# LeadRDRK/ZPack

Measured on AMD Instinct MI355X. Metric: decompressed GiB/s over all entries; % HBM roofline, higher is better.
Workload: dtype u8; 1 GPU; c2_lz4_64k; entries_per_gpu=100000, entries_total=100000, archive_image_bytes_this_rank=3543588472, archive_image_bytes_all_ranks=3543588472, method=lz4, level=0, class_mix=70/20/5/5 text/records/random/runs, parallelism=one batch per rank, no data-path collective, rehearsal_one_card=False, frames_by=liblz4/libzstd of the image, reference writer call sequence

## Files before the change

zpack_amd/csrc/lz4_wave.h:

```cpp
#pragma once
#include "zpk_device.h"
#include "xxh3_device.h"
#include "seq_exec.h"

namespace zpk {

__device__ __noinline__ u32 window_word(const u8* a, const u8* lo, const u8* hi)
{
    if (a >= lo && a + 4 <= hi) return ld32(a);
    u32 v = 0;
    #pragma unroll
    for (int i = 0; i < 4; i++) if (a + i >= lo && a + i < hi) v |= (u32)ld8(a + i) << (8 * i);
    return v;
}

struct ByteWindow {
    u32 w;
    const u8* base;
    const u8* lo;
    const u8* hi;

    __device__ __forceinline__ void load(const u8* p, int lane)
    {
        base = (const u8*)((u64)p & ~(u64)3);
        w = window_word(base + 4 * lane, lo, hi);
    }
    __device__ __forceinline__ u32 byte(const u8* p, int lane)
    {
        u64 d = (u64)(p - base);
        if (d >= 256) { load(p, lane); d = (u64)(p - base); }
        u32 word = (u32)__builtin_amdgcn_readlane((int)w, (int)(d >> 2));
        return (word >> (8 * (d & 3))) & 0xFF;
    }
};

struct DecodeOut { int rc; u64 produced; };

struct Lz4Resume { u64 ip_off, op_off, frame_ip_off, frame_op_off; u32 in_blocks, nframes; };

#ifndef LZ4W_SEG
#define LZ4W_SEG 60u
#endif
static_assert(LZ4W_SEG <= 64u, "the visited-position mask of a segment is one 64-bit word");
#define LZ4W_CHUNK (64u * LZ4W_SEG)
#define LZ4W_SLACK 64u
#ifndef LZ4W_RUNIN
#define LZ4W_RUNIN LZ4W_SEG
#endif

#ifndef LZ4W_SPLIT_FIRST
#define LZ4W_SPLIT_FIRST 0
#endif
#ifndef LZ4W_NREC
#define LZ4W_NREC 576u
#endif
struct alignas(16) Lz4WaveShared {
    u8  stage[LZ4W_CHUNK + LZ4W_SLACK + 16];
    u16 rec[LZ4W_NREC];
};

struct Lz4Bytes {
    lds_cp8 S;
    const u8* g;
    u32 cbase, cend;
    __device__ __forceinline__ u32 at(u32 pos) const
    {
        if (pos < cend) return lds_ld8(S + (pos - cbase));
        return (u32)ld8(g + pos);
    }
    __device__ __forceinline__ u32 at16(u32 pos) const
    {
        if (pos + 1 < cend) return lds_ld16(S + (pos - cbase));
        return at(pos) | (at(pos + 1) << 8);
    }
};

struct Lz4Tok { u32 next, lit_pos, lit, ml, off, flags; };

__device__ __forceinline__ Lz4Tok lz4_token_at(const Lz4Bytes& B, u32 p, u32 C, bool want_offset)
{
    Lz4Tok t; t.flags = 0; t.ml = 0; t.off = 1;
    const u32 tok = B.at(p);
    u32 q = p + 1, lit = tok >> 4;
    if (lit == 15) {
        u32 b;
        do {
            if (q >= C) { t.flags = 1; t.next = C; t.lit = 0; t.lit_pos = q; return t; }
            b = B.at(q++); lit += b;
        } while (b == 255 && lit < 0x7F000000u);
        if (b == 255) { t.flags = 1; t.next = C; t.lit = 0; t.lit_pos = q; return t; }
    }
    t.lit_pos = q; t.lit = lit;
    if (lit > C - q) { t.flags = 1; t.next = C; return t; }
    q += lit;
    if (q == C) { t.flags = 2; t.next = C; return t; }
    if (C - q < 2) { t.flags = 5; t.next = C; return t; }
    if (want_offset) t.off = B.at16(q);
    q += 2;
    u32 ml = tok & 15;
    if (ml == 15) {
        u32 b;
        do {
            if (q >= C) { t.flags = 5; t.next = C; return t; }
            b = B.at(q++); ml += b;
        } while (b == 255 && ml < 0x7F000000u);
        if (b == 255) { t.flags = 5; t.next = C; return t; }
    }
    t.ml = ml + 4;
    t.next = q;
    return t;
}

struct Lz4Quick { u32 lit_pos, lit, ml, next, off, slow; };
__device__ __forceinline__ u32 lt31(u32 a, u32 b) { return (a - b) >> 31; }
__device__ __forceinline__ Lz4Quick lz4_quick(lds_cp8 S, u32 cbase, u32 p, u32 lim)
{
    const lds_cp8 at = S + (p - cbase);
    const u32 tok = lds_ld8(at), b1 = lds_ld8(at + 1);
    const u32 lit4 = tok >> 4, mlc = tok & 15;
    const u32 le = (lit4 + 1) >> 4, me = (mlc + 1) >> 4;
    const u32 lit = lit4 + (b1 & (0u - le));
    const u32 q = 1 + le + lit;
    const u32 b2 = lds_ld8(at + q + 2);
    Lz4Quick r;
    r.off = lds_ld16(at + q);
    r.lit_pos = p + 1 + le; r.lit = lit;
    r.ml = mlc + 4 + (b2 & (0u - me));
    r.next = p + q + 2 + me;
    r.slow = (le & ((b1 + 1) >> 8)) | (me & ((b2 + 1) >> 8)) | lt31(lim, p + q + 3);
    return r;
}

struct Lz4Walk { u32 exit, flags; u64 m; };
template <bool FIRST>
__device__ __forceinline__ Lz4Walk lz4_walk(const Lz4Bytes& B, bool on, u32 from, u32 seg_start, u32 seg_end, u32 C,
                                            const Lz4Walk& old, u32& entry_out, SeqStats& stt)
{
    (void)stt;
    const u32 lim = B.cend < C ? B.cend : C;
    const i32 seg_len = (i32)(seg_end - seg_start), lim_rel = (i32)(lim - seg_start);
    const lds_cp8 base = B.S + (seg_start - B.cbase);
    const bool start_in = on && (i32)(from - seg_start) < seg_len;
    i32 rp = start_in ? (i32)(from - seg_start) : seg_len;
    bool live = start_in, merged = false;
    u32 flags = 0, exit_far = from, far = on && !start_in ? 1u : 0u;
    u64 m = 0;
    for (;;) {
        live = live && rp < seg_len;
        const bool inseg = FIRST ? rp >= 0 : true;
        if (!FIRST) {
            const bool hit = live && ((u32)(old.m >> (rp & 63)) & 1u);
            merged = merged || hit;
            live = live && !hit;
        }
        if (__builtin_amdgcn_ballot_w64(live) == 0) break;
        SEQ_STAT(if (FIRST) stt.hops_first++; else stt.hops_fix++);
        m |= (u64)((live && inseg) ? 1u : 0u) << (rp & 63);
        const lds_cp8 at = base + rp;
        const u32 tok = lds_ld8(at), b1 = lds_ld8(at + 1);
        const u32 lit4 = tok >> 4, mlc = tok & 15;
        const bool l15 = lit4 == 15, m15 = mlc == 15;
        const u32 q = lit4 + 1 + (l15 ? b1 + 1 : 0u);
        const u32 b2 = lds_ld8(at + q + 2);
        const i32 n2 = rp + (i32)q + 2;
        i32 nx = n2 + (m15 ? 1 : 0);
        const bool slow = (l15 && b1 == 255) || (m15 && b2 == 255) || n2 >= lim_rel;
        if (live && slow) {
            SEQ_STAT(stt.slow_hops++);
            const Lz4Tok tt = lz4_token_at(B, seg_start + (u32)rp, C, false);
            nx = (i32)(tt.next - seg_start);
            if (tt.flags && !inseg) nx = 0;
            else if (tt.flags || nx >= seg_len) { flags |= tt.flags; far = 1; exit_far = tt.next; nx = seg_len; }
        }
        rp = live ? nx : rp;
    }
    Lz4Walk w; w.m = m; w.flags = flags; w.exit = far ? exit_far : seg_start + (u32)rp;
    if (merged) {
        const u64 tail = old.m & ~((1ull << (rp & 63)) - 1);
        w.m |= tail;
        w.flags |= old.flags;
        w.exit = old.exit;
    }
    if (!on) w = old;
    entry_out = !FIRST ? from : m ? seg_start + (u32)__ffsll((long long)m) - 1u : w.exit;
    return w;
}

struct Lz4NoEmit { __device__ __forceinline__ int operator()(const SeqBatch&, int, u32) const { return D_OK; } };

template <int COOP = 2, bool EMIT = false, class Emit = Lz4NoEmit>
__device__ inline int lz4_block_wave(Lz4WaveShared& sh, Watchdog& wd, SeqStats& stt, const u8* ip, u32 C, const u8* rd_hi,
                                     u8* dst_lo, u8*& op_io, u8* oend, int lane, Emit emit = Emit())
{
    u8* op = op_io;
    if (C == 0) return D_MALFORMED;
    u32 cpos = 0;
    bool finished = false;
    while (!finished) {
        if (wd.expired()) return D_MALFORMED;
        const u64 tp0 = SEQ_T(); (void)tp0;
        if (cpos >= C) return D_MALFORMED;
        const u32 nst = C - cpos < LZ4W_CHUNK + LZ4W_SLACK ? C - cpos : LZ4W_CHUNK + LZ4W_SLACK;
        const u32 tok_end = C - cpos < LZ4W_CHUNK ? C : cpos + LZ4W_CHUNK;
        wave_mem_fence();
        if (ip + cpos + ((nst + 15u) & ~15u) <= rd_hi) {
            const u8* const g = ip + cpos + 16u * (u32)lane;
            ZPK_LDS u8* const d0 = (ZPK_LDS u8*)sh.stage;
            #pragma unroll
            for (u32 i = 0; i < LZ4W_CHUNK + LZ4W_SLACK; i += WAVE * 16)
                if (i + 16u * (u32)lane < nst) __builtin_amdgcn_global_load_lds((const ZPK_GLOBAL u32*)(g + i), (ZPK_LDS u32*)(d0 + i), 16, 0, 0);
            asm volatile("s_waitcnt vmcnt(0)" ::: "memory");
        } else {
            for (u32 i = (u32)lane * 16; i < nst; i += WAVE * 16) {
                const u8* g = ip + cpos + i;
                if (i + 16 <= nst && g + 16 <= rd_hi) { u128 v = ld128(g); __builtin_memcpy(sh.stage + i, &v, 16); }
                else for (u32 k = i; k < nst && k < i + 16; k++) sh.stage[k] = ld8(ip + cpos + k);
            }
        }
        __builtin_amdgcn_fence(__ATOMIC_ACQ_REL, "workgroup");
        u64 ts = SEQ_T(); (void)ts; SEQ_STAT(stt.t_stage += ts - tp0; stt.chunks++);
        Lz4Bytes B; B.S = to_lds(sh.stage); B.g = ip; B.cbase = cpos; B.cend = cpos + nst;
        const u32 lim = B.cend < C ? B.cend : C;
        const u32 my_start = cpos + (u32)lane * LZ4W_SEG;
        const u32 my_end = my_start + LZ4W_SEG < tok_end ? my_start + LZ4W_SEG : tok_end;
        const bool active = my_start < tok_end;
        u32 my_entry = my_start;
        Lz4Walk w; w.exit = my_start; w.flags = 0; w.m = 0;
        w = lz4_walk<true>(B, active, lane == 0 ? my_start : (my_start - cpos > LZ4W_RUNIN ? my_start - LZ4W_RUNIN : cpos), my_start, my_end, C, w, my_entry, stt);
        SEQ_STAT({ u64 t2 = SEQ_T(); stt.t_walk1 += t2 - ts; ts = t2; });
        for (int iter = 0; iter < 66; iter++) {
            SEQ_STAT(stt.fix_iters++);
            u32 e = (u32)__shfl_up((int)w.exit, 1, 64);
            if (lane == 0) e = cpos;
            const bool changed = active && e != my_entry;
            if (__ballot(changed) == 0) break;
            u32 unused;
            w = lz4_walk<false>(B, changed, e, my_start, my_end, C, w, unused, stt);
            my_entry = changed ? e : my_entry;
        }
        SEQ_STAT({ u64 t2 = SEQ_T(); stt.t_fix += t2 - ts; ts = t2; });
        if (!active) { w.exit = (u32)__shfl((int)w.exit, 63, 64); }
        const u64 lastmask = __ballot(active);
        const int last_lane = 63 - __clzll((long long)lastmask);
        const u32 chain_exit = (u32)__builtin_amdgcn_readlane((int)w.exit, last_lane);
        const u32 fl = (u32)__ballot(active && (w.flags & 1)) != 0 || (__ballot(active && (w.flags & 1)) >> 32) != 0 ? 1u : 0u;
        if (__ballot(active && (w.flags & 2)) != 0) finished = true;
        const u32 my_nseq = active ? (u32)__popcll(w.m) : 0u;
        const u32 x = wave_scan_add(my_nseq);
        const u32 nseq = (u32)__builtin_amdgcn_readlane((int)x, 63);
        SEQ_STAT({ u64 t2 = SEQ_T(); stt.t_emit += t2 - ts; stt.t_parse += t2 - tp0; });
        ZPK_LDS u16* const rec = (ZPK_LDS u16*)sh.rec;
        for (u32 b0 = 0, bstep; b0 < nseq; b0 += bstep) {
            bstep = LZ4W_SPLIT_FIRST && b0 < WAVE ? WAVE / 2 : WAVE;
            const u32 bw = b0 % LZ4W_NREC;
            if (bw == 0) {
                wave_mem_fence();
                u64 m = w.m;
                u32 k = x - my_nseq;
                const u32 rel = my_start - cpos;
                while (m) {
                    const u32 b = (u32)__ffsll((long long)m) - 1u;
                    m &= m - 1;
                    if (k - b0 < LZ4W_NREC) rec[k - b0] = (u16)(rel + b);
                    k++;
                }
                if (active && x == nseq && nseq - b0 < LZ4W_NREC)
                    rec[nseq - b0] = (u16)(w.exit - cpos < LZ4W_CHUNK + LZ4W_SLACK ? w.exit - cpos : LZ4W_CHUNK + LZ4W_SLACK);
                wave_mem_fence();
            }
            const int cnt = (int)(nseq - b0 < bstep ? nseq - b0 : bstep);
            const u64 tq0 = SEQ_T(); (void)tq0;
            SeqBatch q; q.lit = ip; q.lit_lds = SEQ_NO_LDS; q.ll = 0; q.ml = 0; q.off = 1; q.bad = 0;
            u32 tok_pos = cpos;
            if (lane < cnt) {
                const u32 p = cpos + (u32)rec[bw + (u32)lane];
                tok_pos = p;
                const Lz4Quick t = lz4_quick(B.S, B.cbase, p, lim);
                if (!t.slow) {
                    q.lit = ip + t.lit_pos; q.ll = t.lit; q.ml = t.ml; q.off = t.off;
                } else {
                    const Lz4Tok tt = lz4_token_at(B, p, C, true);
                    q.lit = ip + tt.lit_pos; q.ll = tt.lit; q.ml = tt.ml; q.off = tt.off;
                    if (tt.flags & 1) q.bad = (tt.flags & 4) ? 2u : 1u;
                }
                if (q.ll > (1u << 23)) q.ll = 1u << 23;
                if (q.ml > (1u << 23)) q.ml = 1u << 23;
                const u32 lp = (u32)(q.lit - ip);
                if (q.ll <= SEQ_OWN_MAX && lp + q.ll <= B.cend) q.lit_lds = lp - B.cbase;
            }
            SEQ_STAT({ u64 t2 = SEQ_T(); stt.t_parse += t2 - tq0; stt.t_tok += t2 - tq0; });
            u32 dead = 0;
            if constexpr (!EMIT) {
                const u32 nx = bw + (u32)cnt;
                const u32 own = tok_pos - cpos;
#ifdef LZ4W_ROOM_OWN_TOKEN
                (void)nx; const u32 nxt = 0u;
#else
                const u32 nxt = (u32)rec[nx == LZ4W_NREC ? 0u : nx];
#endif
                dead = (u32)__builtin_amdgcn_readfirstlane((int)(nxt > own ? nxt : own));
            }
            int rc;
            if constexpr (EMIT) { (void)dead; rc = emit(q, cnt, (u32)(q.lit - ip)); }
            else rc = seq_exec_batch<true, COOP, SEQ_ASM_LONG_LIT != 0>(q, cnt, op, oend, dst_lo, -1, lane, stt, B.S, to_lds_rw(sh.stage), dead);
            if (rc != D_OK) { op_io = op; return rc; }
        }
        if (fl) return D_MALFORMED;
        if (!finished && chain_exit <= cpos) return D_MALFORMED;
        cpos = chain_exit;
    }
    if (cpos != C) return D_MALFORMED;
    op_io = op;
    return D_OK;
}

template <int COOP = 2>
__device__ inline DecodeOut lz4f_decode_wave(Lz4WaveShared& sh, Watchdog& wd, SeqStats& stt, const u8* src, u64 src_size, const u8* src_lo, const u8* src_hi,
                                             u8* dst, u64 dst_cap, int lane, Lz4Resume* rs = nullptr)
{
    DecodeOut r; r.rc = D_OK; r.produced = 0;
    const u8* ip = src;
    const u8* const iend = src + src_size;
    u8* op = dst;
    u8* const oend = dst + dst_cap;
    bool resume_in_blocks = false, first = true;
    if (rs && (rs->in_blocks || rs->nframes)) {
        ip = src + rs->frame_ip_off; op = dst + rs->frame_op_off;
        resume_in_blocks = rs->in_blocks != 0;
        first = rs->nframes == 0;
    }
    for (;; first = false) {
        if (wd.expired()) { r.rc = D_MALFORMED; return r; }
        if (!first && (ip == iend || op == oend)) break;
        if (rs) { rs->frame_ip_off = (u64)(ip - src); rs->frame_op_off = (u64)(op - dst); if (!resume_in_blocks) rs->in_blocks = 0; }
        if (iend - ip < 7) { r.rc = D_TRUNCATED; r.produced = (u64)(op - dst); return r; }
        const u32 magic = uld32(ip);
        if ((magic & 0xFFFFFFF0u) == 0x184D2A50u) {
            if (iend - ip < 8) { r.rc = D_TRUNCATED; r.produced = (u64)(op - dst); return r; }
            const u64 sz = uld32(ip + 4);
            if ((u64)(iend - ip) - 8 < sz) { r.rc = D_TRUNCATED; r.produced = (u64)(op - dst); return r; }
            ip += 8 + sz;
            if (rs) rs->nframes++;
            continue;
        }
        if (magic != 0x184D2204u) { r.rc = D_MALFORMED; return r; }
        const u32 flg = uld8(ip + 4), bd = uld8(ip + 5);
        const bool indep = (flg >> 5) & 1, bck = (flg >> 4) & 1, has_cs = (flg >> 3) & 1, cck = (flg >> 2) & 1, has_dict = flg & 1;
        if ((flg >> 6) != 1 || (flg & 2)) { r.rc = D_MALFORMED; return r; }
        const u32 hdr = 7 + (has_cs ? 8 : 0) + (has_dict ? 4 : 0);
        if ((u64)(iend - ip) < hdr) { r.rc = D_TRUNCATED; r.produced = (u64)(op - dst); return r; }
        if (bd & 0x8F) { r.rc = D_MALFORMED; return r; }
        const u32 bcode = (bd >> 4) & 7;
        if (bcode < 4) { r.rc = D_MALFORMED; return r; }
        const u64 bmax = (u64)1 << (8 + 2 * bcode);
        u64 content_size = 0;
        if (has_cs) content_size = uni64(ld64(ip + 6));
        {
            u32 h = 0;
            lane0_guard();
            if (lane == 0) h = (xxh32_serial(ip + 4, hdr - 5, 0) >> 8) & 0xFF;
            if (uni(h) != uld8(ip + hdr - 1)) { r.rc = D_MALFORMED; return r; }
        }
        ip += hdr;

        u8* const frame_out = op;
        if (resume_in_blocks) { ip = src + rs->ip_off; op = dst + rs->op_off; resume_in_blocks = false; }
        for (;;) {
            if (wd.expired()) { r.rc = D_MALFORMED; return r; }
            if (rs) { rs->in_blocks = 1; rs->ip_off = (u64)(ip - src); rs->op_off = (u64)(op - dst); }
            if (iend - ip < 4) { r.rc = D_TRUNCATED; r.produced = (u64)(op - dst); return r; }
            const u32 bh = uld32(ip);
            ip += 4;
            if (bh == 0) break;
            const bool raw = bh >> 31;
            const u64 bsz = bh & 0x7FFFFFFFu;
            if (bsz > bmax) { r.rc = D_MALFORMED; return r; }
            if ((u64)(iend - ip) < bsz + (bck ? 4u : 0u)) {
                if (raw && !rs) {
                    u64 n = (u64)(iend - ip); if (n > bsz) n = bsz;
                    bool full = n > (u64)(oend - op);
                    if (full) n = (u64)(oend - op);
                    for (u64 i = (u64)lane * 16; i < n; i += WAVE * 16) gcopy_upto16(op + i, ip + i, (u32)(n - i < 16 ? n - i : 16));
                    op += n;
                    if (full) { r.rc = D_DST_FULL; r.produced = (u64)(op - dst); return r; }
                }
                r.rc = D_TRUNCATED; r.produced = (u64)(op - dst); return r;
            }
            if (bck) {
                u32 h = 0;
                lane0_guard();
                if (lane == 0) h = xxh32_serial(ip, bsz, 0);
                if (uni(h) != uld32(ip + bsz)) { r.rc = D_MALFORMED; return r; }
            }
            if (raw) {
                u64 n = bsz;
                bool full = n > (u64)(oend - op);
                if (full) n = (u64)(oend - op);
                for (u64 i = (u64)lane * 16; i < n; i += WAVE * 16) gcopy_upto16(op + i, ip + i, (u32)(n - i < 16 ? n - i : 16));
                op += n;
                if (full) { r.rc = D_DST_FULL; r.produced = (u64)(op - dst); return r; }
            } else {
                u8* hist_lo = indep ? op : frame_out;
                if ((u64)(op - hist_lo) > 65536) hist_lo = op - 65536;
                u8* bend = oend;
                bool limited = false;
                if ((u64)(oend - op) > bmax) { bend = op + bmax; limited = true; }
                const int rc = lz4_block_wave<COOP>(sh, wd, stt, ip, (u32)bsz, src_hi, hist_lo, op, bend, lane);
                if (rc == D_DST_FULL) {
                    if (limited) { r.rc = D_MALFORMED; return r; }
                    r.rc = D_DST_FULL; r.produced = (u64)(op - dst); return r;
                }
                if (rc != D_OK) { r.rc = D_MALFORMED; return r; }
            }
            wave_mem_fence();
            ip += bsz + (bck ? 4u : 0u);
        }
        if (cck) {
            if (iend - ip < 4) { r.rc = D_TRUNCATED; r.produced = (u64)(op - dst); return r; }
            u32 h = 0;
            lane0_guard();
            if (lane == 0) h = xxh32_serial(frame_out, (u64)(op - frame_out), 0);
            if (uni(h) != uld32(ip)) { r.rc = D_MALFORMED; return r; }
            ip += 4;
        }
        if (has_cs && content_size != (u64)(op - frame_out)) { r.rc = D_MALFORMED; return r; }
        if (rs) { rs->nframes++; rs->in_blocks = 0; rs->frame_ip_off = (u64)(ip - src); rs->frame_op_off = (u64)(op - dst); }
    }
    r.produced = (u64)(op - dst);
    return r;
}

template <int COOP = 0>
__device__ inline bool lz4f_plain_wave(Lz4WaveShared& sh, Watchdog& wd, SeqStats& stt, const u8* src, u64 src_size, const u8* src_hi,
                                       u8* dst, u64 dst_cap, u64 want, int lane)
{
    if (src_size < 11) return false;
    if (uld32(src) != 0x184D2204u) return false;
    const u32 flg = uld8(src + 4), bd = uld8(src + 5);
    if ((flg & 0xD7u) != 0x40u || (bd & 0x8Fu) || ((bd >> 4) & 7u) < 4u) return false;
    const u32 hdr = (flg & 8u) ? 15u : 7u;
    if (src_size < hdr + 4u) return false;
    if ((flg & 8u) && uni64(ld64(src + 6)) != want) return false;
    {
        u32 h = 0;
        lane0_guard();
        if (lane == 0) h = (xxh32_serial(src + 4, hdr - 5, 0) >> 8) & 0xFF;
        if (uni(h) != uld8(src + hdr - 1)) return false;
    }
    const u64 bmax = (u64)1 << (8 + 2 * ((bd >> 4) & 7u));
    const bool indep = (flg >> 5) & 1;
    const u8* ip = src + hdr;
    const u8* const iend = src + src_size;
    u8* op = dst;
    u8* const oend = dst + dst_cap;
    for (;;) {
        if (wd.expired() || iend - ip < 4) return false;
        const u32 bh = uld32(ip);
        ip += 4;
        if (bh == 0) break;
        const u32 bsz = bh & 0x7FFFFFFFu;
        if (bsz > bmax || (u64)(iend - ip) < bsz) return false;
        if (bh >> 31) {
            if (bsz > (u64)(oend - op)) return false;
            for (u32 i = (u32)lane * 16; i < bsz; i += WAVE * 16) gcopy_upto16(op + i, ip + i, bsz - i < 16 ? bsz - i : 16);
            op += bsz;
        } else {
            u8* hist_lo = indep ? op : dst;
            if ((u64)(op - hist_lo) > 65536) hist_lo = op - 65536;
            u8* bend = oend;
            if ((u64)(oend - op) > bmax) bend = op + bmax;
            if (lz4_block_wave<COOP>(sh, wd, stt, ip, bsz, src_hi, hist_lo, op, bend, lane) != D_OK) return false;
        }
        wave_mem_fence();
        ip += bsz;
    }
    return ip == iend && (u64)(op - dst) == want;
}

}
```

Baseline: 675.9 GiB/s.

## Let LZ4 fixpoint walks continue into the next segment with LDS handoff

Restructures the token-boundary fixpoint loop so that a lane whose corrected walk leaves its segment keeps walking into the neighbouring segment. Walk state (mask, exit, flags) is handed between lanes through 16-byte LDS slots, which is meant to shorten serial chains of shuffle-based fix iterations when an entry correction has to ripple across many segments. The merge condition in lz4_walk is also simplified. A separate small tweak pins the input pointer in an SGPR through an empty asm so the slow token path uses a scalar base. In exchange, each iteration does more work and adds LDS traffic and fences, and the rec buffer is reused as scratch.

```diff
diff --git a/zpack_amd/csrc/lz4_wave.h b/zpack_amd/csrc/lz4_wave.h
--- a/zpack_amd/csrc/lz4_wave.h
+++ b/zpack_amd/csrc/lz4_wave.h
@@ -46,6 +46,10 @@
 #define LZ4W_SLACK 64u
 #ifndef LZ4W_RUNIN
 #define LZ4W_RUNIN LZ4W_SEG
+#endif
+
+#ifndef LZ4W_FIX_CONT
+#define LZ4W_FIX_CONT 1
 #endif
 
 #ifndef LZ4W_SPLIT_FIRST
@@ -142,16 +146,14 @@
     const lds_cp8 base = B.S + (seg_start - B.cbase);
     const bool start_in = on && (i32)(from - seg_start) < seg_len;
     i32 rp = start_in ? (i32)(from - seg_start) : seg_len;
-    bool live = start_in, merged = false;
+    bool live = start_in;
     u32 flags = 0, exit_far = from, far = on && !start_in ? 1u : 0u;
     u64 m = 0;
     for (;;) {
         live = live && rp < seg_len;
         const bool inseg = FIRST ? rp >= 0 : true;
         if (!FIRST) {
-            const bool hit = live && ((u32)(old.m >> (rp & 63)) & 1u);
-            merged = merged || hit;
-            live = live && !hit;
+            live = live && !((u32)(old.m >> (rp & 63)) & 1u);
         }
         if (__builtin_amdgcn_ballot_w64(live) == 0) break;
         SEQ_STAT(if (FIRST) stt.hops_first++; else stt.hops_fix++);
@@ -175,7 +177,7 @@
         rp = live ? nx : rp;
     }
     Lz4Walk w; w.m = m; w.flags = flags; w.exit = far ? exit_far : seg_start + (u32)rp;
-    if (merged) {
+    if (!FIRST && rp < seg_len) {
         const u64 tail = old.m & ~((1ull << (rp & 63)) - 1);
         w.m |= tail;
         w.flags |= old.flags;
@@ -228,6 +230,55 @@
         Lz4Walk w; w.exit = my_start; w.flags = 0; w.m = 0;
         w = lz4_walk<true>(B, active, lane == 0 ? my_start : (my_start - cpos > LZ4W_RUNIN ? my_start - LZ4W_RUNIN : cpos), my_start, my_end, C, w, my_entry, stt);
         SEQ_STAT({ u64 t2 = SEQ_T(); stt.t_walk1 += t2 - ts; ts = t2; });
+#if LZ4W_FIX_CONT
+        {
+            static_assert(sizeof(sh.rec) >= 16 * (WAVE + 1), "65 records of 16 bytes (lane 63 reads a slot nobody uses)");
+            const lds_p8 slot = to_lds_rw((u8*)sh.rec) + 16u * (u32)lane;
+            const auto pack = [](const Lz4Walk& a) { u128 v; v.lo = a.m; v.hi = ((u64)a.flags << 32) | a.exit; return v; };
+            const auto unpack = [](const u128& v) { Lz4Walk a; a.m = v.lo; a.exit = (u32)v.hi; a.flags = (u32)(v.hi >> 32); return a; };
+            if (lane == 0) my_entry = w.exit;
+            bool on = false;
+            for (int iter = 0; iter < 2 * 66;) {
+                const bool step2 = iter & 1;
+                const u32 s0 = my_start + (step2 ? LZ4W_SEG : 0u);
+                const u32 s1 = s0 + LZ4W_SEG < C ? s0 + LZ4W_SEG : C;
+                const u32 next_end = s1 + LZ4W_SEG < C ? s1 + LZ4W_SEG : C;
+                u32 from; Lz4Walk old;
+                wave_mem_fence();
+                if (!step2) {
+                    SEQ_STAT(stt.fix_iters++);
+                    from = (u32)__shfl_up((int)w.exit, 1, 64);
+                    on = active && from != my_entry;
+                    if (__ballot(on) == 0) break;
+                    old = w;
+                    lds_st128(slot, pack(w));
+                } else {
+                    from = w.exit;
+                    old = unpack(lds_ld128(slot + 16));
+                    wave_mem_fence();
+                    lds_st128(slot, pack(w));
+                }
+                wave_mem_fence();
+                u32 unused;
+                const Lz4Walk r = lz4_walk<false>(B, on, from, s0, s1, C, old, unused, stt);
+                if (!step2) {
+                    my_entry = on ? from : my_entry;
+                    on = on && r.exit != w.exit && r.exit < next_end && r.exit - cpos < LZ4W_CHUNK;
+                    w = r;
+                    iter += __ballot(on) != 0 ? 1 : 2;
+                } else {
+                    const u32 hn = (u32)__shfl_up((int)from, 1, 64);
+                    const bool got = ((__ballot(on) << 1) >> lane) & 1;
+                    wave_mem_fence();
+                    if (on) lds_st128(slot + 16, pack(r));
+                    wave_mem_fence();
+                    w = unpack(lds_ld128(slot));
+                    my_entry = got ? hn : my_entry;
+                    iter++;
+                }
+            }
+        }
+#else
         for (int iter = 0; iter < 66; iter++) {
             SEQ_STAT(stt.fix_iters++);
             u32 e = (u32)__shfl_up((int)w.exit, 1, 64);
@@ -238,6 +289,7 @@
             w = lz4_walk<false>(B, changed, e, my_start, my_end, C, w, unused, stt);
             my_entry = changed ? e : my_entry;
         }
+#endif
         SEQ_STAT({ u64 t2 = SEQ_T(); stt.t_fix += t2 - ts; ts = t2; });
         if (!active) { w.exit = (u32)__shfl((int)w.exit, 63, 64); }
         const u64 lastmask = __ballot(active);
@@ -249,6 +301,9 @@
         const u32 x = wave_scan_add(my_nseq);
         const u32 nseq = (u32)__builtin_amdgcn_readlane((int)x, 63);
         SEQ_STAT({ u64 t2 = SEQ_T(); stt.t_emit += t2 - ts; stt.t_parse += t2 - tp0; });
+        const u8* ipb = ip;
+        asm volatile("" : "+s"(ipb));
+        Lz4Bytes Bb = B; Bb.g = ipb;
         ZPK_LDS u16* const rec = (ZPK_LDS u16*)sh.rec;
         for (u32 b0 = 0, bstep; b0 < nseq; b0 += bstep) {
             bstep = LZ4W_SPLIT_FIRST && b0 < WAVE ? WAVE / 2 : WAVE;
@@ -270,22 +325,22 @@
             }
             const int cnt = (int)(nseq - b0 < bstep ? nseq - b0 : bstep);
             const u64 tq0 = SEQ_T(); (void)tq0;
-            SeqBatch q; q.lit = ip; q.lit_lds = SEQ_NO_LDS; q.ll = 0; q.ml = 0; q.off = 1; q.bad = 0;
+            SeqBatch q; q.lit = ipb; q.lit_lds = SEQ_NO_LDS; q.ll = 0; q.ml = 0; q.off = 1; q.bad = 0;
             u32 tok_pos = cpos;
             if (lane < cnt) {
                 const u32 p = cpos + (u32)rec[bw + (u32)lane];
                 tok_pos = p;
                 const Lz4Quick t = lz4_quick(B.S, B.cbase, p, lim);
                 if (!t.slow) {
-                    q.lit = ip + t.lit_pos; q.ll = t.lit; q.ml = t.ml; q.off = t.off;
+                    q.lit = ipb + t.lit_pos; q.ll = t.lit; q.ml = t.ml; q.off = t.off;
                 } else {
-                    const Lz4Tok tt = lz4_token_at(B, p, C, true);
-                    q.lit = ip + tt.lit_pos; q.ll = tt.lit; q.ml = tt.ml; q.off = tt.off;
+                    const Lz4Tok tt = lz4_token_at(Bb, p, C, true);
+                    q.lit = ipb + tt.lit_pos; q.ll = tt.lit; q.ml = tt.ml; q.off = tt.off;
                     if (tt.flags & 1) q.bad = (tt.flags & 4) ? 2u : 1u;
                 }
                 if (q.ll > (1u << 23)) q.ll = 1u << 23;
                 if (q.ml > (1u << 23)) q.ml = 1u << 23;
-                const u32 lp = (u32)(q.lit - ip);
+                const u32 lp = (u32)(q.lit - ipb);
                 if (q.ll <= SEQ_OWN_MAX && lp + q.ll <= B.cend) q.lit_lds = lp - B.cbase;
             }
             SEQ_STAT({ u64 t2 = SEQ_T(); stt.t_parse += t2 - tq0; stt.t_tok += t2 - tq0; });
@@ -301,7 +356,7 @@
                 dead = (u32)__builtin_amdgcn_readfirstlane((int)(nxt > own ? nxt : own));
             }
             int rc;
-            if constexpr (EMIT) { (void)dead; rc = emit(q, cnt, (u32)(q.lit - ip)); }
+            if constexpr (EMIT) { (void)dead; rc = emit(q, cnt, (u32)(q.lit - ipb)); }
             else rc = seq_exec_batch<true, COOP, SEQ_ASM_LONG_LIT != 0>(q, cnt, op, oend, dst_lo, -1, lane, stt, B.S, to_lds_rw(sh.stage), dead);
             if (rc != D_OK) { op_io = op; return rc; }
         }
```

New measurement: 699.0 GiB/s (median of 6 runs). 3.4% higher.
